# SobeyMIL/MVOC

Measured on AMD Instinct MI355X. Metric: UNet3D denoising steps/sec, 16x512^2 frames, inversion+compose, higher is better.
Workload: dtype f16

## Files before the change

mvoc_amd/csrc/norm.hip:

```cpp
#include "common.h"

namespace {

struct GnArgs {
  const half_t* x;
  const half_t* x2;
  const half_t* gamma;
  const half_t* beta;
  half_t* out;
  float* ws;
  float* mom_out;
  const float* sums;
  const float* sums2;
  int nslab;
  int inline_final;
  int nsample, R, c, c1, c2, G, cpg, silu;
  int nchunk, rows_per_chunk;
  int CW, RY, npass;
  int aCW, aRY, anpass;
  float eps;
};

__device__ __forceinline__ const half_t* gn_src(const GnArgs& p, long row, int ch) {
  return ch < p.c1 ? p.x + row * p.c1 + ch : p.x2 + row * p.c2 + (ch - p.c1);
}

__global__ __launch_bounds__(256) void gn_partial(const GnArgs p) {
  __shared__ float lsum[2560], lsq[2560];
  const int tid = threadIdx.x;
  const int cx = tid % p.CW, ry = tid / p.CW;
  const int smp = blockIdx.y, chunk = blockIdx.x;
  const int r0 = chunk * p.rows_per_chunk;
  const int r1 = min(r0 + p.rows_per_chunk, p.R);
  const long rowbase = (long)smp * p.R;
  for (int pass = 0; pass < p.npass; ++pass) {
    const int cc = pass * p.CW + cx;
    const bool on = ry < p.RY && cc * 8 < p.c;
    float s[8], q[8];
#pragma unroll
    for (int e = 0; e < 8; ++e) s[e] = q[e] = 0.f;
    if (on) {
      int rr = r0 + ry;
      for (; rr + 3 * p.RY < r1; rr += 4 * p.RY) {
        half8_t v[4];
#pragma unroll
        for (int u = 0; u < 4; ++u) v[u] = *reinterpret_cast<const half8_t*>(gn_src(p, rowbase + rr + u * p.RY, cc * 8));
#pragma unroll
        for (int u = 0; u < 4; ++u)
#pragma unroll
          for (int e = 0; e < 8; ++e) {
            const float f = (float)v[u][e];
            s[e] += f;
            q[e] += f * f;
          }
      }
      for (; rr < r1; rr += p.RY) {
        const half8_t v = *reinterpret_cast<const half8_t*>(gn_src(p, rowbase + rr, cc * 8));
#pragma unroll
        for (int e = 0; e < 8; ++e) {
          const float f = (float)v[e];
          s[e] += f;
          q[e] += f * f;
        }
      }
#pragma unroll
      for (int e = 0; e < 8; ++e) {
        lsum[ry * p.CW * 8 * p.npass + cc * 8 + e] = s[e];
        lsq[ry * p.CW * 8 * p.npass + cc * 8 + e] = q[e];
      }
    }
  }
  __syncthreads();
  if (tid < p.G) {
    float s = 0.f, q = 0.f;
    const int stride = p.CW * 8 * p.npass;
    for (int y = 0; y < p.RY; ++y)
      for (int ch = tid * p.cpg; ch < (tid + 1) * p.cpg; ++ch) {
        s += lsum[y * stride + ch];
        q += lsq[y * stride + ch];
      }
    const float n = (float)(r1 - r0) * p.cpg;
    const float mean = n > 0 ? s / n : 0.f;
    float* o = p.ws + (((long)smp * p.nchunk + chunk) * p.G + tid) * 3;
    o[0] = n;
    o[1] = mean;
    o[2] = fmaxf(q - s * mean, 0.f);
  }
}

struct GnMoments { float n, mean, m2; };
__device__ __forceinline__ void gn_merge(GnMoments& a, float nb, float mb, float m2b) {
  if (nb <= 0.f) return;
  const float nt = a.n + nb, delta = mb - a.mean;
  a.mean += delta * (nb / nt);
  a.m2 += m2b + delta * delta * (a.n * nb / nt);
  a.n = nt;
}

__device__ __forceinline__ void gn_fold_slab(const GnArgs& p, int smp, int g, int sl, float& n, float& mean, float& m2) {
  const int ch0 = g * p.cpg;
  const bool second = ch0 >= p.c1;
  const int cs = second ? p.c2 : p.c1;
  const float* in = (second ? p.sums2 : p.sums) + (((long)smp * p.nslab + sl) * cs + (second ? ch0 - p.c1 : ch0)) * 2;
  float sx = 0.f, sq = 0.f;
  int c = 0;
  if ((p.cpg & 1) == 0) {
    for (; c + 10 <= p.cpg; c += 10) {
      float4 v[5];
#pragma unroll
      for (int u = 0; u < 5; ++u) v[u] = *reinterpret_cast<const float4*>(in + 2 * c + 4 * u);
#pragma unroll
      for (int u = 0; u < 5; ++u) { sx += v[u].x; sq += v[u].y; sx += v[u].z; sq += v[u].w; }
    }
  }
  for (; c < p.cpg; ++c) {
    const float2 v = *reinterpret_cast<const float2*>(in + 2 * c);
    sx += v.x;
    sq += v.y;
  }
  n = 256.f * (float)p.cpg;
  mean = sx / n;
  m2 = fmaxf(sq - sx * mean, 0.f);
}

__global__ __launch_bounds__(1024) void gn_final(const GnArgs p) {
  __shared__ float ln[1024], lmean[1024], lm2[1024];
  const int GL = p.G / gridDim.y;
  const int tid = threadIdx.x, smp = blockIdx.x;
  int lanes = 1;
  while (lanes * 2 * GL <= 1024) lanes *= 2;
  const int gl = tid % GL, lane = tid / GL;
  const int g = blockIdx.y * GL + gl;
  GnMoments acc = {0.f, 0.f, 0.f};
  if (p.sums) {
    if (lane < lanes) {
      for (int sl = lane; sl < p.nslab; sl += lanes) {
        float n, mean, m2;
        gn_fold_slab(p, smp, g, sl, n, mean, m2);
        gn_merge(acc, n, mean, m2);
      }
    }
  } else if (lane < lanes) {
    const float* base = p.ws + ((long)smp * p.nchunk * p.G + g) * 3;
    for (int c0 = lane; c0 < p.nchunk; c0 += lanes * 8) {
      float nb[8], mb[8], qb[8];
#pragma unroll
      for (int u = 0; u < 8; ++u) {
        const int c = c0 + u * lanes;
        nb[u] = 0.f; mb[u] = 0.f; qb[u] = 0.f;
        if (c < p.nchunk) {
          const float* in = base + (long)c * p.G * 3;
          nb[u] = in[0]; mb[u] = in[1]; qb[u] = in[2];
        }
      }
#pragma unroll
      for (int u = 0; u < 8; ++u) gn_merge(acc, nb[u], mb[u], qb[u]);
    }
  }
  ln[tid] = acc.n; lmean[tid] = acc.mean; lm2[tid] = acc.m2;
  __syncthreads();
  for (int half = lanes / 2; half >= 1; half /= 2) {
    if (lane < half) {
      const int o = (lane + half) * GL + gl;
      gn_merge(acc, ln[o], lmean[o], lm2[o]);
      ln[tid] = acc.n; lmean[tid] = acc.mean; lm2[tid] = acc.m2;
    }
    __syncthreads();
  }
  if (lane == 0) {
    if (p.mom_out) {
      float* mo = p.mom_out + ((long)smp * p.G + g) * 3;
      mo[0] = acc.n; mo[1] = acc.mean; mo[2] = acc.m2;
      return;
    }
    float* fin = p.ws + (long)p.nsample * p.nchunk * p.G * 3 + ((long)smp * p.G + g) * 2;
    fin[0] = acc.mean;
    fin[1] = rsqrtf(acc.m2 / acc.n + p.eps);
  }
}

__global__ __launch_bounds__(256) void gn_merge_parts(const float* __restrict__ parts, int nparts, int ng, float eps,
                                                      float* __restrict__ fin) {
  const int i = blockIdx.x * 256 + threadIdx.x;
  if (i >= ng) return;
  GnMoments acc = {0.f, 0.f, 0.f};
  for (int r = 0; r < nparts; ++r) {
    const float* in = parts + ((long)r * ng + i) * 3;
    gn_merge(acc, in[0], in[1], in[2]);
  }
  fin[i * 2] = acc.mean;
  fin[i * 2 + 1] = rsqrtf(acc.m2 / acc.n + eps);
}

template <bool NT>
__global__ __launch_bounds__(256) void gn_apply(const GnArgs p) {
  const int tid = threadIdx.x;
  const int cx = tid % p.aCW, ry = tid / p.aCW;
  const int smp = blockIdx.y, chunk = blockIdx.x;
  const int r0 = chunk * p.rows_per_chunk;
  const int r1 = min(r0 + p.rows_per_chunk, p.R);
  const long rowbase = (long)smp * p.R;
  const float* fin = p.ws + (long)p.nsample * p.nchunk * p.G * 3 + (long)smp * p.G * 2;
  __shared__ float lfin[2 * 256 + 3 * 256];
  if (p.inline_final) {
    const int g = tid % p.G, part = tid / p.G, parts = 256 / p.G;
    GnMoments acc = {0.f, 0.f, 0.f};
    for (int sl = part; sl < p.nslab; sl += parts) {
      float n, mean, m2;
      gn_fold_slab(p, smp, g, sl, n, mean, m2);
      gn_merge(acc, n, mean, m2);
    }
    float* lm = lfin + 2 * 256;
    lm[tid * 3] = acc.n; lm[tid * 3 + 1] = acc.mean; lm[tid * 3 + 2] = acc.m2;
    __syncthreads();
    if (tid < p.G) {
      GnMoments t = {0.f, 0.f, 0.f};
      for (int k = 0; k < parts; ++k) gn_merge(t, lm[(k * p.G + tid) * 3], lm[(k * p.G + tid) * 3 + 1], lm[(k * p.G + tid) * 3 + 2]);
      lfin[tid * 2] = t.mean;
      lfin[tid * 2 + 1] = rsqrtf(t.m2 / t.n + p.eps);
    }
    __syncthreads();
    fin = lfin;
  }
  if (ry >= p.aRY) return;
  for (int pass = 0; pass < p.anpass; ++pass) {
    const int cc = pass * p.aCW + cx;
    if (cc * 8 >= p.c) continue;
    float sc[8], sh[8];
    const half8_t gm = *reinterpret_cast<const half8_t*>(p.gamma + cc * 8);
    const half8_t bt = *reinterpret_cast<const half8_t*>(p.beta + cc * 8);
#pragma unroll
    for (int e = 0; e < 8; ++e) {
      const int g = (cc * 8 + e) / p.cpg;
      const float mean = fin[g * 2], rstd = fin[g * 2 + 1];
      sc[e] = rstd * (float)gm[e];
      sh[e] = (float)bt[e] - mean * sc[e];
    }
    int rr = r0 + ry;
    for (; rr + 3 * p.aRY < r1; rr += 4 * p.aRY) {
      half8_t v[4];
#pragma unroll
      for (int u = 0; u < 4; ++u) {
        const half8_t* src = reinterpret_cast<const half8_t*>(gn_src(p, rowbase + rr + u * p.aRY, cc * 8));
        v[u] = NT ? __builtin_nontemporal_load(src) : *src;
      }
#pragma unroll
      for (int u = 0; u < 4; ++u) {
        half8_t o;
#pragma unroll
        for (int e = 0; e < 8; ++e) {
          float y = r16((float)v[u][e] * sc[e] + sh[e]);
          if (p.silu) y = silu_f(y);
          o[e] = (half_t)y;
        }
        *reinterpret_cast<half8_t*>(p.out + (rowbase + rr + u * p.aRY) * p.c + cc * 8) = o;
      }
    }
    for (; rr < r1; rr += p.aRY) {
      const half8_t v = *reinterpret_cast<const half8_t*>(gn_src(p, rowbase + rr, cc * 8));
      half8_t o;
#pragma unroll
      for (int e = 0; e < 8; ++e) {
        float y = r16((float)v[e] * sc[e] + sh[e]);
        if (p.silu) y = silu_f(y);
        o[e] = (half_t)y;
      }
      *reinterpret_cast<half8_t*>(p.out + (rowbase + rr) * p.c + cc * 8) = o;
    }
  }
}


__global__ __launch_bounds__(256) void gn_fold_xs_kernel(const GnArgs p, const half_t* __restrict__ w, const half_t* __restrict__ bias,
                                                         int n, int k, half_t* __restrict__ wp) {
  const int tile = blockIdx.x, smp = blockIdx.y, tid = threadIdx.x;
  const int nk = k / 16, np = nk + 1;
  const float* fin = p.ws + (long)p.nsample * p.nchunk * p.G * 3 + (long)smp * p.G * 2;
  half_t* out = wp + ((long)smp * (n / 32) + tile) * np * 512;
  for (int q = tid; q < nk * 64; q += 256) {
    const int s_ = q >> 6, l = q & 63;
    const int row = 32 * tile + (l & 31), col = 16 * s_ + 8 * (l >> 5);
    const half8_t wv = *reinterpret_cast<const half8_t*>(w + (long)row * k + col);
    const half8_t gv = *reinterpret_cast<const half8_t*>(p.gamma + col);
    half8_t o;
#pragma unroll
    for (int e = 0; e < 8; ++e) o[e] = (half_t)((float)wv[e] * ((float)gv[e] * fin[2 * ((col + e) / p.cpg) + 1]));
    *reinterpret_cast<half8_t*>(out + (long)q * 8) = o;
  }
  const int r = tid >> 3, part = tid & 7;
  const int row = 32 * tile + r;
  float acc = 0.f;
  for (int col = part * 8; col < k; col += 64) {
    const half8_t wv = *reinterpret_cast<const half8_t*>(w + (long)row * k + col);
    const half8_t gv = *reinterpret_cast<const half8_t*>(p.gamma + col);
    const half8_t bv = *reinterpret_cast<const half8_t*>(p.beta + col);
#pragma unroll
    for (int e = 0; e < 8; ++e) {
      const float* f = fin + 2 * ((col + e) / p.cpg);
      const float wr = (float)(half_t)((float)wv[e] * ((float)gv[e] * f[1]));
      acc += (float)wv[e] * (float)bv[e] - wr * f[0];
    }
  }
  acc += __shfl_xor(acc, 1);
  acc += __shfl_xor(acc, 2);
  acc += __shfl_xor(acc, 4);
  if (part == 0) reinterpret_cast<float*>(out + (long)nk * 512)[r] = acc + (bias ? (float)bias[row] : 0.f);
}

int gn_final_blocks(const GnArgs& a) {
  const int n = a.sums ? a.nslab : a.nchunk;
  return (a.nsample < 16 && n > 64 && a.G % 4 == 0 && a.G >= 8) ? 4 : 1;
}

void gn_geometry(GnArgs& a) {
  const int cchunks = a.c / 8;
  a.CW = cchunks < 256 ? cchunks : 256;
  a.RY = 256 / a.CW;
  a.npass = (cchunks + a.CW - 1) / a.CW;
  a.aCW = a.CW; a.aRY = a.RY; a.anpass = a.npass;
  int want = 2048 / (a.nsample > 0 ? a.nsample : 1);
  if (want < 1) want = 1;
  if (want > 1024) want = 1024;
  int maxchunk = (a.R + a.RY * 4 - 1) / (a.RY * 4);
  if (maxchunk < 1) maxchunk = 1;
  a.nchunk = want < maxchunk ? want : maxchunk;
  a.rows_per_chunk = (a.R + a.nchunk - 1) / a.nchunk;
  a.nchunk = (a.R + a.rows_per_chunk - 1) / a.rows_per_chunk;
}

__global__ __launch_bounds__(256) void ln_kernel(const half_t* __restrict__ x, const half_t* __restrict__ gamma,
                                                 const half_t* __restrict__ beta, half_t* __restrict__ out, long rows,
                                                 int c, float eps) {
  const int lane = threadIdx.x & 63, wave = threadIdx.x >> 6;
  const long row = (long)blockIdx.x * 4 + wave;
  if (row >= rows) return;
  const int nch = c / 8;
  const half_t* xr = x + row * c;
  half8_t v[4];
  float s = 0.f;
#pragma unroll
  for (int i = 0; i < 4; ++i) {
    const int cc = lane + 64 * i;
    if (cc < nch) {
      v[i] = *reinterpret_cast<const half8_t*>(xr + cc * 8);
#pragma unroll
      for (int e = 0; e < 8; ++e) s += (float)v[i][e];
    }
  }
#pragma unroll
  for (int o = 32; o > 0; o >>= 1) s += __shfl_xor(s, o);
  const float mean = s / c;
  float q = 0.f;
#pragma unroll
  for (int i = 0; i < 4; ++i) {
    const int cc = lane + 64 * i;
    if (cc < nch) {
#pragma unroll
      for (int e = 0; e < 8; ++e) {
        const float d = (float)v[i][e] - mean;
        q += d * d;
      }
    }
  }
#pragma unroll
  for (int o = 32; o > 0; o >>= 1) q += __shfl_xor(q, o);
  const float rstd = rsqrtf(q / c + eps);
#pragma unroll
  for (int i = 0; i < 4; ++i) {
    const int cc = lane + 64 * i;
    if (cc < nch) {
      const half8_t gm = *reinterpret_cast<const half8_t*>(gamma + cc * 8);
      const half8_t bt = *reinterpret_cast<const half8_t*>(beta + cc * 8);
      half8_t o;
#pragma unroll
      for (int e = 0; e < 8; ++e) o[e] = (half_t)(((float)v[i][e] - mean) * rstd * (float)gm[e] + (float)bt[e]);
      *reinterpret_cast<half8_t*>(out + row * c + cc * 8) = o;
    }
  }
}

__global__ __launch_bounds__(256) void row_stats_kernel(const half_t* __restrict__ x, float* __restrict__ stats, long rows,
                                                        int c, float eps) {
  const int lane = threadIdx.x & 63, wave = threadIdx.x >> 6;
  const long row = (long)blockIdx.x * 4 + wave;
  if (row >= rows) return;
  const int nch = c / 8;
  const half_t* xr = x + row * c;
  half8_t v[4];
  float s1 = 0.f, s2 = 0.f;
#pragma unroll
  for (int i = 0; i < 4; ++i) {
    const int cc = lane + 64 * i;
    if (cc < nch) {
      v[i] = *reinterpret_cast<const half8_t*>(xr + cc * 8);
#pragma unroll
      for (int e = 0; e < 8; ++e) s1 += (float)v[i][e];
    }
  }
#pragma unroll
  for (int o = 32; o > 0; o >>= 1) s1 += __shfl_xor(s1, o);
  const float mean = s1 / c;
#pragma unroll
  for (int i = 0; i < 4; ++i) {
    const int cc = lane + 64 * i;
    if (cc < nch) {
#pragma unroll
      for (int e = 0; e < 8; ++e) {
        const float dv = (float)v[i][e] - mean;
        s2 += dv * dv;
      }
    }
  }
#pragma unroll
  for (int o = 32; o > 0; o >>= 1) s2 += __shfl_xor(s2, o);
  if (lane == 0) {
    stats[2 * row] = mean;
    stats[2 * row + 1] = rsqrtf(s2 / c + eps);
  }
}

}

namespace {
__global__ __launch_bounds__(256) void softmax_rows_kernel(half_t* __restrict__ x, long rows, int cols) {
  const int lane = threadIdx.x & 63, wave = threadIdx.x >> 6;
  const long row = (long)blockIdx.x * 4 + wave;
  if (row >= rows) return;
  half_t* xr = x + row * cols;
  const int nch = cols / 8;
  float mx = -3.0e38f;
  for (int c = lane; c < nch; c += 64) {
    const half8_t v = *reinterpret_cast<const half8_t*>(xr + c * 8);
#pragma unroll
    for (int e = 0; e < 8; ++e) mx = fmaxf(mx, (float)v[e]);
  }
#pragma unroll
  for (int o = 32; o > 0; o >>= 1) mx = fmaxf(mx, __shfl_xor(mx, o));
  float sum = 0.f;
  for (int c = lane; c < nch; c += 64) {
    const half8_t v = *reinterpret_cast<const half8_t*>(xr + c * 8);
#pragma unroll
    for (int e = 0; e < 8; ++e) sum += __expf((float)v[e] - mx);
  }
#pragma unroll
  for (int o = 32; o > 0; o >>= 1) sum += __shfl_xor(sum, o);
  const float inv = 1.0f / sum;
  for (int c = lane; c < nch; c += 64) {
    half8_t v = *reinterpret_cast<const half8_t*>(xr + c * 8);
#pragma unroll
    for (int e = 0; e < 8; ++e) v[e] = (half_t)(__expf((float)v[e] - mx) * inv);
    *reinterpret_cast<half8_t*>(xr + c * 8) = v;
  }
}
}

extern "C" int mvoc_softmax_rows_f16(void* x, int64_t rows, int32_t cols, void* stream) {
  MVOC_REQUIRE(x && rows > 0 && cols > 0 && cols % 8 == 0 && ((uintptr_t)x & 15) == 0, -1, "softmax_rows: bad args (cols %% 8, 16-byte aligned)");
  hipStream_t s = (hipStream_t)stream;
  MvocProfScope prof(MVOC_FAM_MISC, s, 4.0 * rows * cols);
  hipLaunchKernelGGL(softmax_rows_kernel, dim3((unsigned)((rows + 3) / 4)), dim3(256), 0, s, (half_t*)x, (long)rows, cols);
  return mvoc_check_launch("softmax_rows_kernel");
}

extern "C" int mvoc_row_stats_f16(const void* x, void* stats, int64_t rows, int32_t c, float eps, void* stream) {
  MVOC_REQUIRE(x && stats && rows > 0 && c >= 8 && c % 8 == 0 && c <= 2048, -1, "row_stats: bad args (c %% 8 == 0, c <= 2048)");
  hipStream_t s = (hipStream_t)stream;
  MvocProfScope prof(MVOC_FAM_LN, s, 2.0 * (double)rows * c);
  const long nblk = (rows + 3) / 4;
  MVOC_REQUIRE(nblk < 0x7fffffffL, -2, "row_stats: too many rows");
  hipLaunchKernelGGL(row_stats_kernel, dim3((unsigned)nblk), dim3(256), 0, s, (const half_t*)x, (float*)stats, (long)rows, c, eps);
  return mvoc_check_launch("row_stats_kernel");
}

namespace {
__global__ __launch_bounds__(256) void row_stats_from_moments_kernel(const float* __restrict__ mom, float* __restrict__ stats, long rows,
                                                                     int ld, int n, int tile_w, float eps) {
  const long r = (long)blockIdx.x * 256 + threadIdx.x;
  if (r >= rows) return;
  const float2* in = reinterpret_cast<const float2*>(mom) + r * ld;
  float cnt = 0.f, mean = 0.f, m2 = 0.f;
  for (int t = 0; t * tile_w < n; ++t) {
    const float2 v = in[t];
    const float nb = (float)min(tile_w, n - t * tile_w);
    const float mb = v.x / nb;
    const float m2b = fmaxf(v.y - v.x * mb, 0.f);
    const float nt = cnt + nb, delta = mb - mean;
    mean += delta * (nb / nt);
    m2 += m2b + delta * delta * (cnt * nb / nt);
    cnt = nt;
  }
  reinterpret_cast<float2*>(stats)[r] = float2{mean, rsqrtf(m2 / cnt + eps)};
}
}

extern "C" int mvoc_row_stats_from_moments_f32(const void* moments, int64_t rows, int32_t ld, int32_t n, int32_t tile_w, float eps,
                                               void* out_stats, void* stream) {
  MVOC_REQUIRE(moments && out_stats && rows > 0 && n > 0 && (tile_w == 256 || tile_w == 320) && ld >= (n + tile_w - 1) / tile_w, -1,
               "row_stats_from_moments: bad args (tile_w 256 | 320, ld >= ceil(n / tile_w))");
  hipStream_t s = (hipStream_t)stream;
  MvocProfScope prof(MVOC_FAM_LN, s, (double)rows * (8.0 * ((n + tile_w - 1) / tile_w) + 8.0));
  const long nblk = (rows + 255) / 256;
  MVOC_REQUIRE(nblk < 0x7fffffffL, -2, "row_stats_from_moments: too many rows");
  hipLaunchKernelGGL(row_stats_from_moments_kernel, dim3((unsigned)nblk), dim3(256), 0, s, (const float*)moments, (float*)out_stats,
                     (long)rows, ld, n, tile_w, eps);
  return mvoc_check_launch("row_stats_from_moments_kernel");
}

extern "C" size_t mvoc_groupnorm_workspace_bytes(int32_t nsample, int32_t rows_per_sample, int32_t c, int32_t groups) {
  GnArgs a;
  memset(&a, 0, sizeof(a));
  a.nsample = nsample; a.R = rows_per_sample; a.c = c; a.G = groups;
  if (nsample <= 0 || rows_per_sample <= 0 || c < 8 || groups <= 0) return 0;
  gn_geometry(a);
  return ((size_t)nsample * a.nchunk * groups * 3 + (size_t)nsample * groups * 2) * sizeof(float);
}

namespace {
int gn_setup(const mvoc_gn_desc* d, bool need_affine, GnArgs& a) {
  MVOC_REQUIRE(d && d->x && d->workspace && (!need_affine || (d->gamma && d->beta && d->out)), -1, "groupnorm: null operand");
  MVOC_REQUIRE(d->nsample > 0 && d->rows_per_sample > 0, -1, "groupnorm: empty problem");
  MVOC_REQUIRE(d->c % 8 == 0 && d->c1 % 8 == 0 && d->c <= 2560 && d->groups > 0 && d->groups <= 256 &&
                   d->c % d->groups == 0,
               -2, "groupnorm: unsupported channels %d (c1 %d) / groups %d", d->c, d->c1, d->groups);
  MVOC_REQUIRE(d->x2 || d->c1 == d->c, -1, "groupnorm: c1 < c needs a second source");
  MVOC_REQUIRE(d->nsample <= 65535, -2, "groupnorm: too many samples");
  memset(&a, 0, sizeof(a));
  a.x = (const half_t*)d->x; a.x2 = (const half_t*)d->x2; a.gamma = (const half_t*)d->gamma;
  a.beta = (const half_t*)d->beta; a.out = (half_t*)d->out; a.ws = (float*)d->workspace;
  a.nsample = d->nsample; a.R = d->rows_per_sample; a.c = d->c; a.c1 = d->c1; a.c2 = d->c - d->c1;
  a.G = d->groups; a.cpg = d->c / d->groups; a.silu = d->silu; a.eps = d->eps;
  gn_geometry(a);
  const size_t need = mvoc_groupnorm_workspace_bytes(d->nsample, d->rows_per_sample, d->c, d->groups);
  MVOC_REQUIRE(d->workspace_bytes >= need, -1, "groupnorm: workspace %zu < %zu bytes", d->workspace_bytes, need);
  return 0;
}
}

extern "C" int mvoc_groupnorm_moments_f16(const mvoc_gn_desc* d, void* moments, void* stream) {
  GnArgs a;
  if (int rc = gn_setup(d, false, a)) return rc;
  MVOC_REQUIRE(moments, -1, "groupnorm_moments: null output");
  a.mom_out = (float*)moments;
  hipStream_t s = (hipStream_t)stream;
  MvocProfScope prof(MVOC_FAM_GN, s, 2.0 * (double)d->nsample * d->rows_per_sample * d->c);
  hipLaunchKernelGGL(gn_partial, dim3(a.nchunk, a.nsample), dim3(256), 0, s, a);
  hipLaunchKernelGGL(gn_final, dim3(a.nsample, gn_final_blocks(a)), dim3(1024), 0, s, a);
  return mvoc_check_launch("groupnorm_moments");
}

extern "C" int mvoc_groupnorm_apply_moments_f16(const mvoc_gn_desc* d, const void* parts, int32_t nparts, void* stream) {
  GnArgs a;
  if (int rc = gn_setup(d, true, a)) return rc;
  MVOC_REQUIRE(parts && nparts > 0, -1, "groupnorm_apply_moments: no statistics");
  hipStream_t s = (hipStream_t)stream;
  MvocProfScope prof(MVOC_FAM_GN, s, 2.0 * 2.0 * (double)d->nsample * d->rows_per_sample * d->c);
  const int ng = a.nsample * a.G;
  float* fin = a.ws + (long)a.nsample * a.nchunk * a.G * 3;
  hipLaunchKernelGGL(gn_merge_parts, dim3((ng + 255) / 256), dim3(256), 0, s, (const float*)parts, nparts, ng, a.eps, fin);
  hipLaunchKernelGGL(gn_apply<false>, dim3(a.nchunk, a.nsample), dim3(256), 0, s, a);
  return mvoc_check_launch("groupnorm_apply_moments");
}

extern "C" int mvoc_groupnorm_f16(const mvoc_gn_desc* d, void* stream) {
  GnArgs a;
  if (int rc = gn_setup(d, true, a)) return rc;
  hipStream_t s = (hipStream_t)stream;
  MvocProfScope prof(MVOC_FAM_GN, s, 2.0 * 2.0 * (double)d->nsample * d->rows_per_sample * d->c);
  dim3 grid(a.nchunk, a.nsample);
  if (d->chan_sums) {
    MVOC_REQUIRE(d->rows_per_sample % 256 == 0 && (!d->x2 || d->chan_sums2) && a.c1 % a.cpg == 0, -2,
                 "groupnorm: chan_sums needs rows_per_sample %% 256 == 0, sums of both sources, and groups that do not straddle them");
    a.sums = (const float*)d->chan_sums;
    a.sums2 = (const float*)d->chan_sums2;
    a.nslab = d->rows_per_sample / 256;
    static const long inline_max = getenv("MVOC_GN_INLINE_BYTES") ? atol(getenv("MVOC_GN_INLINE_BYTES")) : 49152;
    a.inline_final = (long)a.nslab * a.c * 8 <= inline_max && a.nslab <= 16 && 256 % a.G == 0;
  } else {
    hipLaunchKernelGGL(gn_partial, grid, dim3(256), 0, s, a);
  }
  if (!a.inline_final) hipLaunchKernelGGL(gn_final, dim3(a.nsample, gn_final_blocks(a)), dim3(1024), 0, s, a);
  static const long nt_min = getenv("MVOC_GN_NT_BYTES") ? atol(getenv("MVOC_GN_NT_BYTES")) : (160L << 20);
  if ((long)d->nsample * d->rows_per_sample * d->c * 2 >= nt_min) hipLaunchKernelGGL(gn_apply<true>, grid, dim3(256), 0, s, a);
  else hipLaunchKernelGGL(gn_apply<false>, grid, dim3(256), 0, s, a);
  return mvoc_check_launch("groupnorm");
}


extern "C" int mvoc_groupnorm_fold_xs_f16(const mvoc_gn_desc* d, const void* w, const void* bias, int32_t n, int32_t k, void* wp_sets,
                                          void* stream) {
  GnArgs a;
  if (int rc = gn_setup(d, false, a)) return rc;
  MVOC_REQUIRE(w && wp_sets && d->gamma && d->beta, -1, "groupnorm_fold_xs: null operand");
  MVOC_REQUIRE(d->x2 == nullptr && k == d->c && n > 0 && n % 32 == 0 && k % 16 == 0 && a.cpg >= 1, -2,
               "groupnorm_fold_xs: single source, k == c, n %% 32 == 0, k %% 16 == 0");
  hipStream_t s = (hipStream_t)stream;
  MvocProfScope prof(MVOC_FAM_GN, s, (d->chan_sums ? 0.0 : 2.0 * (double)d->nsample * d->rows_per_sample * d->c) +
                                         2.0 * 2.0 * (double)d->nsample * n * k);
  if (d->chan_sums) {
    MVOC_REQUIRE(d->rows_per_sample % 256 == 0, -2, "groupnorm_fold_xs: chan_sums needs rows_per_sample %% 256 == 0");
    a.sums = (const float*)d->chan_sums;
    a.nslab = d->rows_per_sample / 256;
  } else {
    hipLaunchKernelGGL(gn_partial, dim3(a.nchunk, a.nsample), dim3(256), 0, s, a);
  }
  hipLaunchKernelGGL(gn_final, dim3(a.nsample, gn_final_blocks(a)), dim3(1024), 0, s, a);
  hipLaunchKernelGGL(gn_fold_xs_kernel, dim3(n / 32, a.nsample), dim3(256), 0, s, a, (const half_t*)w, (const half_t*)bias, (int)n,
                     (int)k, (half_t*)wp_sets);
  return mvoc_check_launch("groupnorm_fold_xs");
}

extern "C" int mvoc_layernorm_f16(const void* x, const void* gamma, const void* beta, void* out, int64_t rows, int32_t c,
                                  float eps, void* stream) {
  MVOC_REQUIRE(x && gamma && beta && out, -1, "layernorm: null operand");
  MVOC_REQUIRE(rows > 0 && c >= 8 && c % 8 == 0 && c <= 2048, -2, "layernorm: unsupported c %d", c);
  hipStream_t s = (hipStream_t)stream;
  MvocProfScope prof(MVOC_FAM_LN, s, 2.0 * 2.0 * (double)rows * c);
  const long nblk = (rows + 3) / 4;
  MVOC_REQUIRE(nblk < 0x7fffffffL, -2, "layernorm: too many rows");
  hipLaunchKernelGGL(ln_kernel, dim3((unsigned)nblk), dim3(256), 0, s, (const half_t*)x, (const half_t*)gamma,
                     (const half_t*)beta, (half_t*)out, (long)rows, c, eps);
  return mvoc_check_launch("ln_kernel");
}
```

mvoc_amd/csrc/stem.hip:

```cpp
#include "common.h"

namespace {

__global__ void timestep_embedding_kernel(const float* __restrict__ t, int nb, int dim, half_t* __restrict__ out) {
  const int i = blockIdx.x * blockDim.x + threadIdx.x;
  const int half = dim / 2;
  if (i >= nb * dim) return;
  const int b = i / dim, j = i % dim;
  const int k = j < half ? j : j - half;
  const float freq = expf(-logf(10000.0f) * (float)k / (float)half);
  const float ang = t[b] * freq;
  out[i] = (half_t)(j < half ? cosf(ang) : sinf(ang));
}

__global__ void act_kernel(const half_t* __restrict__ x, half_t* __restrict__ out, long n, int act) {
  const long i = (long)blockIdx.x * blockDim.x + threadIdx.x;
  if (i >= n) return;
  const float v = (float)x[i];
  out[i] = (half_t)(act == MVOC_ACT_SILU ? silu_f(v) : act == MVOC_ACT_GELU ? gelu_erf_f(v) : v);
}

__global__ void add_kernel(const half_t* __restrict__ a, const half_t* __restrict__ b, half_t* __restrict__ out, long n) {
  const long i = (long)blockIdx.x * blockDim.x + threadIdx.x;
  if (i >= n) return;
  out[i] = (half_t)((float)a[i] + (float)b[i]);
}

__global__ void conv3x3_small_kernel(const half_t* __restrict__ x, const half_t* __restrict__ w,
                                     const half_t* __restrict__ bias, half_t* __restrict__ out, int nimg, int h, int wd,
                                     int cin, int cout, int stride, int ho, int wo, int silu) {
  const long i = (long)blockIdx.x * blockDim.x + threadIdx.x;
  const long total = (long)nimg * ho * wo * cout;
  if (i >= total) return;
  const int co = (int)(i % cout);
  long pix = i / cout;
  const int ox = (int)(pix % wo);
  pix /= wo;
  const int oy = (int)(pix % ho);
  const int img = (int)(pix / ho);
  float acc = 0.f;
  for (int ky = 0; ky < 3; ++ky) {
    const int iy = oy * stride + ky - 1;
    if (iy < 0 || iy >= h) continue;
    for (int kx = 0; kx < 3; ++kx) {
      const int ix = ox * stride + kx - 1;
      if (ix < 0 || ix >= wd) continue;
      const half_t* xp = x + (((long)img * h + iy) * wd + ix) * cin;
      const half_t* wp = w + ((long)co * 9 + ky * 3 + kx) * cin;
      for (int c = 0; c < cin; ++c) acc += (float)xp[c] * (float)wp[c];
    }
  }
  float v = r16(acc + (bias ? (float)bias[co] : 0.f));
  if (silu) v = silu_f(v);
  out[i] = (half_t)v;
}

__global__ void avgpool_kernel(const half_t* __restrict__ x, half_t* __restrict__ out, int nimg, int h, int w, int c,
                               int oh, int ow) {
  const long i = (long)blockIdx.x * blockDim.x + threadIdx.x;
  const long total = (long)nimg * oh * ow * c;
  if (i >= total) return;
  const int ch = (int)(i % c);
  long pix = i / c;
  const int ox = (int)(pix % ow);
  pix /= ow;
  const int oy = (int)(pix % oh);
  const int img = (int)(pix / oh);
  const int y0 = (oy * h) / oh, y1 = ((oy + 1) * h + oh - 1) / oh;
  const int x0 = (ox * w) / ow, x1 = ((ox + 1) * w + ow - 1) / ow;
  float s = 0.f;
  for (int y = y0; y < y1; ++y)
    for (int xx = x0; xx < x1; ++xx) s += (float)x[(((long)img * h + y) * w + xx) * c + ch];
  out[i] = (half_t)(s / (float)((y1 - y0) * (x1 - x0)));
}

__global__ void ncfhw_to_tokens_kernel(const half_t* __restrict__ x, half_t* __restrict__ out, int b, int c, int f, int hw,
                                       int ldo, int coff) {
  const long i = (long)blockIdx.x * blockDim.x + threadIdx.x;
  const long total = (long)b * f * hw;
  if (i >= total) return;
  const int p = (int)(i % hw);
  const long bf = i / hw;
  const int fi = (int)(bf % f), bi = (int)(bf / f);
  for (int ch = 0; ch < c; ++ch) out[i * ldo + coff + ch] = x[(((long)bi * c + ch) * f + fi) * hw + p];
}

__global__ void tokens_to_ncfhw_kernel(const half_t* __restrict__ x, half_t* __restrict__ out, int b, int c, int f, int hw,
                                       int ld) {
  const long i = (long)blockIdx.x * blockDim.x + threadIdx.x;
  const long total = (long)b * c * f * hw;
  if (i >= total) return;
  const int p = (int)(i % hw);
  long r = i / hw;
  const int fi = (int)(r % f);
  r /= f;
  const int ch = (int)(r % c);
  const int bi = (int)(r / c);
  out[i] = x[(((long)bi * f + fi) * hw + p) * ld + ch];
}

struct Enc4Params {
  half_t ln_g[4], ln_b[4], wq[32], wk[32], wv[32], wo[32], bo[4], w1[64], b1[16], w2[64], b2[4];
};

__device__ __forceinline__ void enc4_ln(const half_t* xp, const Enc4Params& P, float* y) {
  float v[4], mean = 0.f;
#pragma unroll
  for (int c = 0; c < 4; ++c) { v[c] = (float)xp[c]; mean += v[c]; }
  mean *= 0.25f;
  float var = 0.f;
#pragma unroll
  for (int c = 0; c < 4; ++c) var += (v[c] - mean) * (v[c] - mean);
  const float rstd = rsqrtf(var * 0.25f + 1e-5f);
#pragma unroll
  for (int c = 0; c < 4; ++c) y[c] = r16((v[c] - mean) * rstd * (float)P.ln_g[c] + (float)P.ln_b[c]);
}

__global__ void temporal_encoder4_kernel(const half_t* __restrict__ x, const Enc4Params* __restrict__ params,
                                         half_t* __restrict__ out, int b, int f, int hw, int ldo, int coff) {
  __shared__ Enc4Params P;
  for (int i = threadIdx.x; i < (int)(sizeof(Enc4Params) / sizeof(half_t)); i += blockDim.x)
    reinterpret_cast<half_t*>(&P)[i] = reinterpret_cast<const half_t*>(params)[i];
  __syncthreads();
  const long idx = (long)blockIdx.x * blockDim.x + threadIdx.x;
  const long total = (long)b * f * hw;
  if (idx >= total) return;
  const int p = (int)(idx % hw);
  const long bf = idx / hw;
  const int bi = (int)(bf / f);
  const half_t* xi = x + idx * 4;
  float yi[4], q[8];
  enc4_ln(xi, P, yi);
#pragma unroll
  for (int o = 0; o < 8; ++o) {
    float s = 0.f;
#pragma unroll
    for (int c = 0; c < 4; ++c) s += yi[c] * (float)P.wq[o * 4 + c];
    q[o] = r16(s);
  }
  float m[2] = {-INFINITY, -INFINITY}, l[2] = {0.f, 0.f}, acc[8] = {0, 0, 0, 0, 0, 0, 0, 0};
  for (int j = 0; j < f; ++j) {
    const half_t* xj = x + (((long)bi * f + j) * hw + p) * 4;
    float yj[4], k[8], v[8];
    enc4_ln(xj, P, yj);
#pragma unroll
    for (int o = 0; o < 8; ++o) {
      float sk = 0.f, sv = 0.f;
#pragma unroll
      for (int c = 0; c < 4; ++c) {
        sk += yj[c] * (float)P.wk[o * 4 + c];
        sv += yj[c] * (float)P.wv[o * 4 + c];
      }
      k[o] = r16(sk);
      v[o] = r16(sv);
    }
#pragma unroll
    for (int hd = 0; hd < 2; ++hd) {
      float s = 0.f;
#pragma unroll
      for (int d = 0; d < 4; ++d) s += q[hd * 4 + d] * k[hd * 4 + d];
      s *= 0.5f;
      const float mn = fmaxf(m[hd], s);
      const float a = __expf(m[hd] - mn), pj = __expf(s - mn);
      l[hd] = l[hd] * a + pj;
#pragma unroll
      for (int d = 0; d < 4; ++d) acc[hd * 4 + d] = acc[hd * 4 + d] * a + pj * v[hd * 4 + d];
      m[hd] = mn;
    }
  }
  float att[8];
#pragma unroll
  for (int o = 0; o < 8; ++o) att[o] = r16(acc[o] / l[o >> 2]);
  float h1[4];
#pragma unroll
  for (int c = 0; c < 4; ++c) {
    float s = 0.f;
#pragma unroll
    for (int o = 0; o < 8; ++o) s += att[o] * (float)P.wo[c * 8 + o];
    h1[c] = r16(r16(s + (float)P.bo[c]) + (float)xi[c]);
  }
  float ff[16];
#pragma unroll
  for (int o = 0; o < 16; ++o) {
    float s = 0.f;
#pragma unroll
    for (int c = 0; c < 4; ++c) s += h1[c] * (float)P.w1[o * 4 + c];
    ff[o] = r16(gelu_erf_f(r16(s + (float)P.b1[o])));
  }
#pragma unroll
  for (int c = 0; c < 4; ++c) {
    float s = 0.f;
#pragma unroll
    for (int o = 0; o < 16; ++o) s += ff[o] * (float)P.w2[c * 16 + o];
    out[idx * ldo + coff + c] = (half_t)(r16(s + (float)P.b2[c]) + h1[c]);
  }
}

__global__ void delay_kernel(long ticks) {
  const long t0 = __builtin_amdgcn_s_memrealtime();
  while ((long)__builtin_amdgcn_s_memrealtime() - t0 < ticks) __builtin_amdgcn_s_sleep(32);
}

inline unsigned nblk(long n, int bs = 256) { return (unsigned)((n + bs - 1) / bs); }

__global__ __launch_bounds__(256) void clip_patches_kernel(const half_t* __restrict__ x, half_t* __restrict__ out, int size, int patch,
                                                           int kpad, long total) {
  const long i = (long)blockIdx.x * 256 + threadIdx.x;
  if (i >= total) return;
  const int g = size / patch;
  const int k = (int)(i % kpad);
  const long row = i / kpad;
  half_t v = (half_t)0.f;
  if (k < 3 * patch * patch) {
    const int c = k / (patch * patch), py = (k / patch) % patch, px = k % patch;
    const int gx = (int)(row % g), gy = (int)((row / g) % g);
    const long b = row / ((long)g * g);
    v = x[((b * 3 + c) * size + gy * patch + py) * (long)size + gx * patch + px];
  }
  out[i] = v;
}

__global__ __launch_bounds__(256) void clip_embed_kernel(const half_t* __restrict__ table, const int* __restrict__ ids,
                                                         const half_t* __restrict__ cls, const half_t* __restrict__ pos,
                                                         half_t* __restrict__ out, int T, int c8n, long total) {
  const long i = (long)blockIdx.x * 256 + threadIdx.x;
  if (i >= total) return;
  const int c8 = (int)(i % c8n);
  const long row = i / c8n;
  const int t = (int)(row % T);
  const half_t* src;
  if (ids) src = table + ((long)ids[row] * c8n + c8) * 8;
  else if (t == 0) src = cls + c8 * 8;
  else src = table + (((row / T) * (T - 1) + t - 1) * c8n + c8) * 8;
  const half8_t a = *reinterpret_cast<const half8_t*>(src);
  const half8_t b = *reinterpret_cast<const half8_t*>(pos + ((long)t * c8n + c8) * 8);
  half8_t o;
#pragma unroll
  for (int e = 0; e < 8; ++e) o[e] = (half_t)((float)a[e] + (float)b[e]);
  reinterpret_cast<half8_t*>(out)[i] = o;
}

}

extern "C" int mvoc_timestep_embedding_f16(const float* t_dev, int32_t nb, int32_t dim, void* out, void* stream) {
  MVOC_REQUIRE(t_dev && out && nb > 0 && dim > 0 && dim % 2 == 0, -1, "timestep_embedding: bad args");
  hipStream_t s = (hipStream_t)stream;
  MvocProfScope prof(MVOC_FAM_MISC, s, 2.0 * nb * dim);
  hipLaunchKernelGGL(timestep_embedding_kernel, dim3(nblk((long)nb * dim)), dim3(256), 0, s, t_dev, nb, dim, (half_t*)out);
  return mvoc_check_launch("timestep_embedding_kernel");
}

extern "C" int mvoc_act_f16(const void* x, void* out, int64_t n, int32_t act, void* stream) {
  MVOC_REQUIRE(x && out && n > 0, -1, "act: bad args");
  hipStream_t s = (hipStream_t)stream;
  MvocProfScope prof(MVOC_FAM_MISC, s, 4.0 * n);
  hipLaunchKernelGGL(act_kernel, dim3(nblk(n)), dim3(256), 0, s, (const half_t*)x, (half_t*)out, (long)n, act);
  return mvoc_check_launch("act_kernel");
}

extern "C" int mvoc_add_f16(const void* a, const void* b, void* out, int64_t n, void* stream) {
  MVOC_REQUIRE(a && b && out && n > 0, -1, "add: bad args");
  hipStream_t s = (hipStream_t)stream;
  MvocProfScope prof(MVOC_FAM_MISC, s, 6.0 * n);
  hipLaunchKernelGGL(add_kernel, dim3(nblk(n)), dim3(256), 0, s, (const half_t*)a, (const half_t*)b, (half_t*)out, (long)n);
  return mvoc_check_launch("add_kernel");
}

extern "C" int mvoc_conv3x3_small_f16(const void* x, const void* w, const void* bias, void* out, int32_t nimg, int32_t h,
                                      int32_t wd, int32_t cin, int32_t cout, int32_t stride, int32_t silu, void* stream) {
  MVOC_REQUIRE(x && w && out && nimg > 0 && h > 0 && wd > 0 && cin > 0 && cout > 0 && (stride == 1 || stride == 2), -1,
               "conv3x3_small: bad args");
  const int ho = (h + 2 - 3) / stride + 1, wo = (wd + 2 - 3) / stride + 1;
  const long total = (long)nimg * ho * wo * cout;
  hipStream_t s = (hipStream_t)stream;
  MvocProfScope prof(MVOC_FAM_MISC, s, 2.0 * ((double)nimg * h * wd * cin + total));
  hipLaunchKernelGGL(conv3x3_small_kernel, dim3(nblk(total)), dim3(256), 0, s, (const half_t*)x, (const half_t*)w,
                     (const half_t*)bias, (half_t*)out, nimg, h, wd, cin, cout, stride, ho, wo, silu);
  return mvoc_check_launch("conv3x3_small_kernel");
}

__global__ void conv1x1_small_kernel(const half_t* __restrict__ x, const half_t* __restrict__ w, const half_t* __restrict__ bias,
                                     half_t* __restrict__ out, long rows, int cin, int cout) {
  const long i = (long)blockIdx.x * blockDim.x + threadIdx.x;
  if (i >= rows * cout) return;
  const int co = (int)(i % cout);
  const long r = i / cout;
  float acc = 0.f;
  for (int c = 0; c < cin; ++c) acc += (float)x[r * cin + c] * (float)w[co * cin + c];
  out[i] = (half_t)(acc + (bias ? (float)bias[co] : 0.f));
}

__global__ void image_to_tokens_kernel(const half_t* __restrict__ x, half_t* __restrict__ out, int n, int c, int hw) {
  const long i = (long)blockIdx.x * blockDim.x + threadIdx.x;
  if (i >= (long)n * hw * c) return;
  const int ch = (int)(i % c);
  const long px = i / c;
  const int img = (int)(px / hw), p = (int)(px % hw);
  out[i] = x[((long)img * c + ch) * hw + p];
}
__global__ void tokens_to_image_kernel(const half_t* __restrict__ x, half_t* __restrict__ out, int n, int c, int hw, int ld) {
  const long i = (long)blockIdx.x * blockDim.x + threadIdx.x;
  if (i >= (long)n * c * hw) return;
  const int p = (int)(i % hw);
  const long t = i / hw;
  const int ch = (int)(t % c), img = (int)(t / c);
  out[i] = x[((long)img * hw + p) * ld + ch];
}

__global__ void gaussian_sample_kernel(const half_t* __restrict__ mean, const half_t* __restrict__ logvar,
                                       const half_t* __restrict__ noise, half_t* __restrict__ out, long n) {
  const long i = (long)blockIdx.x * blockDim.x + threadIdx.x;
  if (i >= n) return;
  const float lv = fminf(fmaxf((float)logvar[i], -30.0f), 20.0f);
  const float sd = r16(expf(r16(0.5f * lv)));
  out[i] = (half_t)((float)mean[i] + r16(sd * (float)noise[i]));
}
__global__ void scale_kernel(const half_t* __restrict__ x, half_t* __restrict__ out, long n, float s) {
  const long i = (long)blockIdx.x * blockDim.x + threadIdx.x;
  if (i >= n) return;
  float p = s * (float)x[i];
  asm volatile("" : "+v"(p));
  out[i] = (half_t)p;
}

extern "C" int mvoc_gaussian_sample_f16(const void* mean, const void* logvar, const void* noise, void* out, int64_t n, void* stream) {
  MVOC_REQUIRE(mean && logvar && noise && out && n > 0, -1, "gaussian_sample: bad args");
  hipStream_t s = (hipStream_t)stream;
  MvocProfScope prof(MVOC_FAM_MISC, s, 8.0 * n);
  hipLaunchKernelGGL(gaussian_sample_kernel, dim3(nblk(n)), dim3(256), 0, s, (const half_t*)mean, (const half_t*)logvar,
                     (const half_t*)noise, (half_t*)out, (long)n);
  return mvoc_check_launch("gaussian_sample_kernel");
}

extern "C" int mvoc_clip_patches_f16(const void* pixels, void* out, int32_t nimg, int32_t size, int32_t patch, int32_t kpad,
                                     void* stream) {
  MVOC_REQUIRE(pixels && out && nimg > 0 && patch > 0 && size > 0 && size % patch == 0 && kpad >= 3 * patch * patch, -1,
               "clip_patches: bad args");
  const long total = (long)nimg * (size / patch) * (size / patch) * kpad;
  hipStream_t s = (hipStream_t)stream;
  MvocProfScope prof(MVOC_FAM_MISC, s, 4.0 * total);
  hipLaunchKernelGGL(clip_patches_kernel, dim3(nblk(total)), dim3(256), 0, s, (const half_t*)pixels, (half_t*)out, size, patch, kpad, total);
  return mvoc_check_launch("clip_patches_kernel");
}

extern "C" int mvoc_clip_embed_f16(const void* table, const int32_t* ids, const void* cls, const void* pos, void* out, int64_t rows,
                                   int32_t t, int32_t c, void* stream) {
  MVOC_REQUIRE(table && pos && out && rows > 0 && t > 0 && rows % t == 0 && c > 0 && c % 8 == 0 && (ids || cls), -1,
               "clip_embed: bad args (c %% 8, rows %% t, ids or cls)");
  const long total = rows * (c / 8);
  hipStream_t s = (hipStream_t)stream;
  MvocProfScope prof(MVOC_FAM_MISC, s, 6.0 * rows * c);
  hipLaunchKernelGGL(clip_embed_kernel, dim3(nblk(total)), dim3(256), 0, s, (const half_t*)table, (const int*)ids, (const half_t*)cls,
                     (const half_t*)pos, (half_t*)out, t, c / 8, total);
  return mvoc_check_launch("clip_embed_kernel");
}

extern "C" int mvoc_scale_f16(const void* x, void* out, int64_t n, double scale, void* stream) {
  MVOC_REQUIRE(x && out && n > 0, -1, "scale: bad args");
  hipStream_t s = (hipStream_t)stream;
  MvocProfScope prof(MVOC_FAM_MISC, s, 4.0 * n);
  hipLaunchKernelGGL(scale_kernel, dim3(nblk(n)), dim3(256), 0, s, (const half_t*)x, (half_t*)out, (long)n, (float)scale);
  return mvoc_check_launch("scale_kernel");
}

extern "C" int mvoc_conv1x1_small_f16(const void* x, const void* w, const void* bias, void* out, int64_t rows, int32_t cin,
                                      int32_t cout, void* stream) {
  MVOC_REQUIRE(x && w && out && rows > 0 && cin > 0 && cout > 0 && cin <= 64 && cout <= 64, -1, "conv1x1_small: bad args");
  hipStream_t s = (hipStream_t)stream;
  MvocProfScope prof(MVOC_FAM_MISC, s, 2.0 * rows * (cin + cout));
  hipLaunchKernelGGL(conv1x1_small_kernel, dim3(nblk(rows * cout)), dim3(256), 0, s, (const half_t*)x, (const half_t*)w,
                     (const half_t*)bias, (half_t*)out, (long)rows, cin, cout);
  return mvoc_check_launch("conv1x1_small_kernel");
}

extern "C" int mvoc_image_to_tokens_f16(const void* x, void* out, int32_t n, int32_t c, int32_t hw, void* stream) {
  MVOC_REQUIRE(x && out && n > 0 && c > 0 && hw > 0, -1, "image_to_tokens: bad args");
  hipStream_t s = (hipStream_t)stream;
  MvocProfScope prof(MVOC_FAM_MISC, s, 4.0 * n * c * hw);
  hipLaunchKernelGGL(image_to_tokens_kernel, dim3(nblk((long)n * c * hw)), dim3(256), 0, s, (const half_t*)x, (half_t*)out, n, c, hw);
  return mvoc_check_launch("image_to_tokens_kernel");
}

extern "C" int mvoc_tokens_to_image_f16(const void* x, void* out, int32_t n, int32_t c, int32_t hw, int32_t ld, void* stream) {
  MVOC_REQUIRE(x && out && n > 0 && c > 0 && hw > 0 && ld >= c, -1, "tokens_to_image: bad args");
  hipStream_t s = (hipStream_t)stream;
  MvocProfScope prof(MVOC_FAM_MISC, s, 4.0 * n * c * hw);
  hipLaunchKernelGGL(tokens_to_image_kernel, dim3(nblk((long)n * c * hw)), dim3(256), 0, s, (const half_t*)x, (half_t*)out, n, c, hw, ld);
  return mvoc_check_launch("tokens_to_image_kernel");
}

__global__ void resize8_pass_kernel(const uint8_t* __restrict__ in, uint8_t* __restrict__ out, const int* __restrict__ bounds,
                                    const int* __restrict__ kk, int ksize, long nimg, int olen, int other, long in_img, long out_img,
                                    long in_si, long in_so, long out_si, long out_so) {
  const long i = (long)blockIdx.x * blockDim.x + threadIdx.x;
  if (i >= nimg * olen * other) return;
  const int xx = (int)(i % olen);
  const long t = i / olen;
  const int o = (int)(t % other);
  const long img = t / other;
  const int xmin = bounds[2 * xx], n = bounds[2 * xx + 1];
  const uint8_t* src = in + img * in_img + (long)o * in_so + (long)xmin * in_si;
  int acc = 1 << 21;
  for (int x = 0; x < n; ++x) acc += (int)src[(long)x * in_si] * kk[xx * ksize + x];
  acc >>= 22;
  out[img * out_img + (long)o * out_so + (long)xx * out_si] = (uint8_t)(acc < 0 ? 0 : acc > 255 ? 255 : acc);
}
__global__ void mask_finish_kernel(const uint8_t* __restrict__ v, half_t* __restrict__ fl, uint8_t* __restrict__ bl, long n) {
  const long i = (long)blockIdx.x * blockDim.x + threadIdx.x;
  if (i >= n) return;
  const int x = v[i];
  fl[i] = (half_t)((float)x / 255.0f);
  bl[i] = x > 10 ? 1 : 0;
}

extern "C" int mvoc_mask_resize_u8(const void* in, void* tmp, void* out, int32_t n, int32_t H, int32_t W, int32_t h, int32_t w,
                                   const int32_t* bounds_h, const int32_t* kk_h, int32_t ksize_h, const int32_t* bounds_v,
                                   const int32_t* kk_v, int32_t ksize_v, void* stream) {
  MVOC_REQUIRE(in && tmp && out && bounds_h && kk_h && bounds_v && kk_v && n > 0 && H > 0 && W > 0 && h > 0 && w > 0, -1, "mask_resize: bad args");
  hipStream_t s = (hipStream_t)stream;
  MvocProfScope prof(MVOC_FAM_MISC, s, (double)n * H * W + 2.0 * n * H * w + (double)n * h * w);
  hipLaunchKernelGGL(resize8_pass_kernel, dim3(nblk((long)n * H * w)), dim3(256), 0, s, (const uint8_t*)in, (uint8_t*)tmp, bounds_h, kk_h,
                     ksize_h, (long)n, w, H, (long)H * W, (long)H * w, 1L, (long)W, 1L, (long)w);
  hipLaunchKernelGGL(resize8_pass_kernel, dim3(nblk((long)n * h * w)), dim3(256), 0, s, (const uint8_t*)tmp, (uint8_t*)out, bounds_v, kk_v,
                     ksize_v, (long)n, h, w, (long)H * w, (long)h * w, (long)w, 1L, (long)w, 1L);
  return mvoc_check_launch("resize8_pass_kernel");
}

extern "C" int mvoc_mask_finish(const void* v, void* float_mask, void* bool_mask, int64_t n, void* stream) {
  MVOC_REQUIRE(v && float_mask && bool_mask && n > 0, -1, "mask_finish: bad args");
  hipStream_t s = (hipStream_t)stream;
  MvocProfScope prof(MVOC_FAM_MISC, s, 4.0 * n);
  hipLaunchKernelGGL(mask_finish_kernel, dim3(nblk(n)), dim3(256), 0, s, (const uint8_t*)v, (half_t*)float_mask, (uint8_t*)bool_mask, (long)n);
  return mvoc_check_launch("mask_finish_kernel");
}

__global__ void permute_rows_kernel(const half_t* __restrict__ x, half_t* __restrict__ out, int d1, int d2, int d3, long s0, long s1,
                                    long s2, long s3, int c8n, long total) {
  const long i = (long)blockIdx.x * blockDim.x + threadIdx.x;
  if (i >= total) return;
  const int c8 = (int)(i % c8n);
  long r = i / c8n;
  const int i3 = (int)(r % d3); r /= d3;
  const int i2 = (int)(r % d2); r /= d2;
  const int i1 = (int)(r % d1);
  const long i0 = r / d1;
  const long src = i0 * s0 + i1 * s1 + i2 * s2 + i3 * s3;
  reinterpret_cast<half8_t*>(out)[i] = *reinterpret_cast<const half8_t*>(x + (src * c8n + c8) * 8);
}

extern "C" int mvoc_permute_rows_f16(const void* x, void* out, const int64_t* dims4, const int64_t* strides4, int32_t c, void* stream) {
  MVOC_REQUIRE(x && out && dims4 && strides4 && c > 0 && c % 8 == 0, -1, "permute_rows: bad args (c %% 8)");
  for (int k = 0; k < 4; ++k) MVOC_REQUIRE(dims4[k] > 0 && dims4[k] < (1 << 30), -1, "permute_rows: bad dim");
  const long total = (long)dims4[0] * dims4[1] * dims4[2] * dims4[3] * (c / 8);
  hipStream_t s = (hipStream_t)stream;
  MvocProfScope prof(MVOC_FAM_MISC, s, 32.0 * total);
  hipLaunchKernelGGL(permute_rows_kernel, dim3(nblk(total)), dim3(256), 0, s, (const half_t*)x, (half_t*)out, (int)dims4[1], (int)dims4[2],
                     (int)dims4[3], (long)strides4[0], (long)strides4[1], (long)strides4[2], (long)strides4[3], c / 8, total);
  return mvoc_check_launch("permute_rows_kernel");
}

extern "C" int mvoc_adaptive_avgpool_f16(const void* x, void* out, int32_t nimg, int32_t h, int32_t w, int32_t c,
                                         int32_t oh, int32_t ow, void* stream) {
  MVOC_REQUIRE(x && out && nimg > 0 && h > 0 && w > 0 && c > 0 && oh > 0 && ow > 0, -1, "avgpool: bad args");
  const long total = (long)nimg * oh * ow * c;
  hipStream_t s = (hipStream_t)stream;
  MvocProfScope prof(MVOC_FAM_MISC, s, 2.0 * ((double)nimg * h * w * c + total));
  hipLaunchKernelGGL(avgpool_kernel, dim3(nblk(total)), dim3(256), 0, s, (const half_t*)x, (half_t*)out, nimg, h, w, c, oh,
                     ow);
  return mvoc_check_launch("avgpool_kernel");
}

extern "C" int mvoc_ncfhw_to_tokens_f16(const void* x, void* out, int32_t b, int32_t c, int32_t f, int32_t hw, int32_t ldo,
                                        int32_t coff, void* stream) {
  MVOC_REQUIRE(x && out && b > 0 && c > 0 && f > 0 && hw > 0 && ldo >= coff + c, -1, "ncfhw_to_tokens: bad args");
  hipStream_t s = (hipStream_t)stream;
  MvocProfScope prof(MVOC_FAM_MISC, s, 4.0 * b * c * f * hw);
  hipLaunchKernelGGL(ncfhw_to_tokens_kernel, dim3(nblk((long)b * f * hw)), dim3(256), 0, s, (const half_t*)x,
                     (half_t*)out, b, c, f, hw, ldo, coff);
  return mvoc_check_launch("ncfhw_to_tokens_kernel");
}

extern "C" int mvoc_tokens_to_ncfhw_f16(const void* x, void* out, int32_t b, int32_t c, int32_t f, int32_t hw, int32_t ld,
                                        void* stream) {
  MVOC_REQUIRE(x && out && b > 0 && c > 0 && f > 0 && hw > 0 && ld >= c, -1, "tokens_to_ncfhw: bad args");
  hipStream_t s = (hipStream_t)stream;
  MvocProfScope prof(MVOC_FAM_MISC, s, 4.0 * b * c * f * hw);
  hipLaunchKernelGGL(tokens_to_ncfhw_kernel, dim3(nblk((long)b * c * f * hw)), dim3(256), 0, s, (const half_t*)x,
                     (half_t*)out, b, c, f, hw, ld);
  return mvoc_check_launch("tokens_to_ncfhw_kernel");
}

extern "C" int mvoc_temporal_encoder4_f16(const void* x, const void* params, void* out, int32_t b, int32_t f, int32_t hw,
                                          int32_t ldo, int32_t coff, void* stream) {
  MVOC_REQUIRE(x && params && out && b > 0 && f > 0 && hw > 0 && ldo >= coff + 4, -1, "temporal_encoder4: bad args");
  hipStream_t s = (hipStream_t)stream;
  MvocProfScope prof(MVOC_FAM_MISC, s, 16.0 * b * f * hw);
  hipLaunchKernelGGL(temporal_encoder4_kernel, dim3(nblk((long)b * f * hw)), dim3(256), 0, s, (const half_t*)x,
                     (const Enc4Params*)params, (half_t*)out, b, f, hw, ldo, coff);
  return mvoc_check_launch("temporal_encoder4_kernel");
}

extern "C" int mvoc_delay_us(int64_t us, void* stream) {
  MVOC_REQUIRE(us >= 0 && us <= 2000000, -1, "delay_us: out of range");
  hipLaunchKernelGGL(delay_kernel, dim3(1), dim3(64), 0, (hipStream_t)stream, (long)us * 100);
  return mvoc_check_launch("delay_kernel");
}
```

Baseline: 21.51.

## Add lane-parallel groupnorm final reduction and vectorized elementwise add kernel

```diff
diff --git a/mvoc_amd/csrc/norm.hip b/mvoc_amd/csrc/norm.hip
--- a/mvoc_amd/csrc/norm.hip
+++ b/mvoc_amd/csrc/norm.hip
@@ -179,6 +179,95 @@
   }
 }
 
+__device__ __forceinline__ void gn_fold_slab_round(const GnArgs& p, int smp, int g, int sl, float& n, float& mean, float& m2) {
+  const int ch0 = g * p.cpg;
+  const bool second = ch0 >= p.c1;
+  const int cs = second ? p.c2 : p.c1;
+  const float* in = (second ? p.sums2 : p.sums) + (((long)smp * p.nslab + sl) * cs + (second ? ch0 - p.c1 : ch0)) * 2;
+  float sx = 0.f, sq = 0.f;
+  if ((p.cpg & 1) == 0) {
+    const int np = p.cpg >> 1;
+    for (int c0 = 0; c0 < np; c0 += 20) {
+      float4 v[20];
+#pragma unroll
+      for (int u = 0; u < 20; ++u) {
+        v[u] = float4{0.f, 0.f, 0.f, 0.f};
+        if (c0 + u < np) v[u] = *reinterpret_cast<const float4*>(in + 4 * (c0 + u));
+      }
+#pragma unroll
+      for (int u = 0; u < 20; ++u) { sx += v[u].x; sq += v[u].y; sx += v[u].z; sq += v[u].w; }
+    }
+  } else {
+    for (int c0 = 0; c0 < p.cpg; c0 += 8) {
+      float2 v[8];
+#pragma unroll
+      for (int u = 0; u < 8; ++u) {
+        v[u] = float2{0.f, 0.f};
+        if (c0 + u < p.cpg) v[u] = *reinterpret_cast<const float2*>(in + 2 * (c0 + u));
+      }
+#pragma unroll
+      for (int u = 0; u < 8; ++u) { sx += v[u].x; sq += v[u].y; }
+    }
+  }
+  n = 256.f * (float)p.cpg;
+  mean = sx / n;
+  m2 = fmaxf(sq - sx * mean, 0.f);
+}
+
+__global__ __launch_bounds__(256) void gn_final_round(const GnArgs p, const int lanes) {
+  __shared__ float lw[4][3];
+  const int tid = threadIdx.x, smp = blockIdx.x;
+  const int GL = 256 / lanes;
+  const int gl = tid / lanes, lane = tid % lanes;
+  const int g = blockIdx.y * GL + gl;
+  GnMoments acc = {0.f, 0.f, 0.f};
+  if (p.sums) {
+    for (int sl = lane; sl < p.nslab; sl += lanes) {
+      float n, mean, m2;
+      gn_fold_slab_round(p, smp, g, sl, n, mean, m2);
+      gn_merge(acc, n, mean, m2);
+    }
+  } else {
+    const float* base = p.ws + ((long)smp * p.nchunk * p.G + g) * 3;
+    for (int c0 = lane; c0 < p.nchunk; c0 += lanes * 4) {
+      float nb[4], mb[4], qb[4];
+#pragma unroll
+      for (int u = 0; u < 4; ++u) {
+        const int c = c0 + u * lanes;
+        nb[u] = 0.f; mb[u] = 0.f; qb[u] = 0.f;
+        if (c < p.nchunk) {
+          const float* in = base + (long)c * p.G * 3;
+          nb[u] = in[0]; mb[u] = in[1]; qb[u] = in[2];
+        }
+      }
+#pragma unroll
+      for (int u = 0; u < 4; ++u) gn_merge(acc, nb[u], mb[u], qb[u]);
+    }
+  }
+  const int wl = lanes < 64 ? lanes : 64;
+  for (int off = wl >> 1; off >= 1; off >>= 1) {
+    const float nb = __shfl_down(acc.n, off), mb = __shfl_down(acc.mean, off), qb = __shfl_down(acc.m2, off);
+    gn_merge(acc, nb, mb, qb);
+  }
+  if (lanes > 64) {
+    const int wave = tid >> 6;
+    if ((tid & 63) == 0) { lw[wave][0] = acc.n; lw[wave][1] = acc.mean; lw[wave][2] = acc.m2; }
+    __syncthreads();
+    if (lane == 0)
+      for (int k = 1; k < lanes / 64; ++k) gn_merge(acc, lw[wave + k][0], lw[wave + k][1], lw[wave + k][2]);
+  }
+  if (lane == 0) {
+    if (p.mom_out) {
+      float* mo = p.mom_out + ((long)smp * p.G + g) * 3;
+      mo[0] = acc.n; mo[1] = acc.mean; mo[2] = acc.m2;
+      return;
+    }
+    float* fin = p.ws + (long)p.nsample * p.nchunk * p.G * 3 + ((long)smp * p.G + g) * 2;
+    fin[0] = acc.mean;
+    fin[1] = rsqrtf(acc.m2 / acc.n + p.eps);
+  }
+}
+
 __global__ __launch_bounds__(256) void gn_merge_parts(const float* __restrict__ parts, int nparts, int ng, float eps,
                                                       float* __restrict__ fin) {
   const int i = blockIdx.x * 256 + threadIdx.x;
@@ -310,6 +399,19 @@
 int gn_final_blocks(const GnArgs& a) {
   const int n = a.sums ? a.nslab : a.nchunk;
   return (a.nsample < 16 && n > 64 && a.G % 4 == 0 && a.G >= 8) ? 4 : 1;
+}
+
+void gn_launch_final(const GnArgs& a, hipStream_t s) {
+  const char* e = getenv("MVOC_GN_FAST_FINAL");
+  if (e && e[0] == '0') {
+    hipLaunchKernelGGL(gn_final, dim3(a.nsample, gn_final_blocks(a)), dim3(1024), 0, s, a);
+    return;
+  }
+  const int n = a.sums ? a.nslab : a.nchunk;
+  int lanes = 1;
+  while (lanes < n && lanes < 256) lanes *= 2;
+  while (a.G % (256 / lanes)) lanes *= 2;
+  hipLaunchKernelGGL(gn_final_round, dim3(a.nsample, a.G / (256 / lanes)), dim3(256), 0, s, a, lanes);
 }
 
 void gn_geometry(GnArgs& a) {
@@ -544,7 +646,7 @@
   hipStream_t s = (hipStream_t)stream;
   MvocProfScope prof(MVOC_FAM_GN, s, 2.0 * (double)d->nsample * d->rows_per_sample * d->c);
   hipLaunchKernelGGL(gn_partial, dim3(a.nchunk, a.nsample), dim3(256), 0, s, a);
-  hipLaunchKernelGGL(gn_final, dim3(a.nsample, gn_final_blocks(a)), dim3(1024), 0, s, a);
+  gn_launch_final(a, s);
   return mvoc_check_launch("groupnorm_moments");
 }
 
@@ -578,7 +680,7 @@
   } else {
     hipLaunchKernelGGL(gn_partial, grid, dim3(256), 0, s, a);
   }
-  if (!a.inline_final) hipLaunchKernelGGL(gn_final, dim3(a.nsample, gn_final_blocks(a)), dim3(1024), 0, s, a);
+  if (!a.inline_final) gn_launch_final(a, s);
   static const long nt_min = getenv("MVOC_GN_NT_BYTES") ? atol(getenv("MVOC_GN_NT_BYTES")) : (160L << 20);
   if ((long)d->nsample * d->rows_per_sample * d->c * 2 >= nt_min) hipLaunchKernelGGL(gn_apply<true>, grid, dim3(256), 0, s, a);
   else hipLaunchKernelGGL(gn_apply<false>, grid, dim3(256), 0, s, a);
@@ -603,7 +705,7 @@
   } else {
     hipLaunchKernelGGL(gn_partial, dim3(a.nchunk, a.nsample), dim3(256), 0, s, a);
   }
-  hipLaunchKernelGGL(gn_final, dim3(a.nsample, gn_final_blocks(a)), dim3(1024), 0, s, a);
+  gn_launch_final(a, s);
   hipLaunchKernelGGL(gn_fold_xs_kernel, dim3(n / 32, a.nsample), dim3(256), 0, s, a, (const half_t*)w, (const half_t*)bias, (int)n,
                      (int)k, (half_t*)wp_sets);
   return mvoc_check_launch("groupnorm_fold_xs");
diff --git a/mvoc_amd/csrc/stem.hip b/mvoc_amd/csrc/stem.hip
--- a/mvoc_amd/csrc/stem.hip
+++ b/mvoc_amd/csrc/stem.hip
@@ -24,6 +24,19 @@
   const long i = (long)blockIdx.x * blockDim.x + threadIdx.x;
   if (i >= n) return;
   out[i] = (half_t)((float)a[i] + (float)b[i]);
+}
+
+__global__ __launch_bounds__(256) void add8_kernel(const half_t* __restrict__ a, const half_t* __restrict__ b, half_t* __restrict__ out, long n) {
+  const long n8 = n >> 3;
+  for (long i = (long)blockIdx.x * 256 + threadIdx.x; i < n8; i += (long)gridDim.x * 256) {
+    const half8_t va = reinterpret_cast<const half8_t*>(a)[i], vb = reinterpret_cast<const half8_t*>(b)[i];
+    half8_t o;
+#pragma unroll
+    for (int e = 0; e < 8; ++e) o[e] = (half_t)((float)va[e] + (float)vb[e]);
+    reinterpret_cast<half8_t*>(out)[i] = o;
+  }
+  const long t = (n8 << 3) + threadIdx.x;
+  if (blockIdx.x == 0 && t < n) out[t] = (half_t)((float)a[t] + (float)b[t]);
 }
 
 __global__ void conv3x3_small_kernel(const half_t* __restrict__ x, const half_t* __restrict__ w,
@@ -262,6 +275,12 @@
   MVOC_REQUIRE(a && b && out && n > 0, -1, "add: bad args");
   hipStream_t s = (hipStream_t)stream;
   MvocProfScope prof(MVOC_FAM_MISC, s, 6.0 * n);
+  if ((((uintptr_t)a | (uintptr_t)b | (uintptr_t)out) & 15) == 0) {
+    const long nb = (n / 8 + 255) / 256;
+    hipLaunchKernelGGL(add8_kernel, dim3((unsigned)(nb < 1 ? 1 : nb > 4096 ? 4096 : nb)), dim3(256), 0, s, (const half_t*)a,
+                       (const half_t*)b, (half_t*)out, (long)n);
+    return mvoc_check_launch("add8_kernel");
+  }
   hipLaunchKernelGGL(add_kernel, dim3(nblk(n)), dim3(256), 0, s, (const half_t*)a, (const half_t*)b, (half_t*)out, (long)n);
   return mvoc_check_launch("add_kernel");
 }
```

New measurement: 21.51 (median of 2 runs). About the same (+0.0%).
